# masafumiendo/benchnav

Hardware: AMD Instinct MI355X
Metric: MPPI solve-steps/sec (K=1024,T=50,256x256 map) (higher is better)
Workload: dtype f32

## Files before the change

### benchnav_amd/csrc/mppi_capi.cpp

```cpp
#include "../../include/benchnav_mppi.h"
#include "mppi_kernels.h"
#include "bn_host.h"
#include "astar_dwa.h"
#include "clrrt_view.h"

#include <algorithm>
#include <atomic>
#include <cmath>
#include <chrono>
#include <cstdarg>
#include <cstdio>
#include <cstdlib>
#include <cstring>
#include <cerrno>
#include <sys/stat.h>
#include <fcntl.h>
#include <sys/file.h>
#include <unistd.h>
#include <dlfcn.h>
#include <hsa/hsa.h>
#include <hsa/hsa_ext_amd.h>
#include <rccl/rccl.h>
#include <map>
#include <mutex>
// ... 83 lines not shown
    hipStream_t stream = nullptr;
    bool own_stream = false;
    int n_maps = 1;
    uint64_t solves = 0;
    bool map_set = false, goal_set = false;
    uint64_t map_epoch = 0, map_epoch_at_solve = 0;
    bool pipelined = false;
    bool slow_path = false;
    bool tail_pending = false;
    float *d_map = nullptr, *d_state = nullptr, *d_goal = nullptr, *d_mean = nullptr, *d_eps = nullptr;
    float *d_X = nullptr, *d_U = nullptr, *d_w = nullptr, *d_cost_out = nullptr;
    float *d_cost[kSlots] = {}, *d_part[kSlots] = {}, *d_state_copy[kSlots] = {};
    float *d_ustar = nullptr, *d_xstar = nullptr, *d_stats = nullptr, *d_scratch = nullptr;
    float *d_mean_used = nullptr;
    int *d_idx = nullptr;
    const float *last_eps = nullptr;
    bn::EpsMode last_mode = bn::kEpsPhilox;
    float *d_slip_std = nullptr;
    float *d_ustar2[kSlots] = {}, *d_stats2[kSlots] = {};
    bool ticket_overlap = false;
    std::vector<float> dwa_stage;
    int *d_ticket = nullptr;
    float *d_gpart = nullptr;
    int n_cus = 256;
    size_t resident_wgs = 1024;
    int n_streams = 1;
    hipStream_t xstream[kMaxStreams - 1] = {};
    std::vector<hipStream_t> parked;
    hipEvent_t ev_fork = nullptr, ev_join[kMaxStreams - 1] = {};
    hipEvent_t ev_guard[kMaxStreams] = {};
    unsigned long long *d_flags = nullptr;
    bool role_overlap = false;
    unsigned long long *d_gran[kSlots] = {};
    float *d_Xalt[kMaxStreams - 1] = {}, *d_Ualt[kMaxStreams - 1] = {};
    unsigned long long pub[kSlots] = {};
    unsigned long long tails = 0;
    bool prev_published = false;
    bool overlap_used = false;
    bool overlap_off = false;
    int *h_err = nullptr, *d_err = nullptr;
    unsigned long long *h_mail = nullptr, *d_mail = nullptr;
    float *d_mean_snap = nullptr;
    float *d_state_snaps = nullptr;
    size_t snap_cap = 0;
    size_t snap_slot = 0;
    bool arm_state_snap = false;
    struct BatchRec { int32_t n; const float *states; const float *eps; bn_noise_kind noise; int32_t eps_ring; int64_t eps_stride; bool episode; const float *z; };
    std::vector<BatchRec> journal;
    bool journal_lost = false;
    bool arm_snap = false;
    bool replaying = false, last_batch_overlapped = false;
    uint64_t journal_solves0 = 0, recoveries = 0;
    struct OvTune { double best[2] = {0, 0}, last[2] = {0, 0}, ema[2] = {0, 0}; int chosen = 0, explore = 0, slow_run = 0; uint64_t windows[2] = {0, 0}, since_explore = 0, switches = 0; } tune;
    struct OvSample { bool valid = false; std::chrono::steady_clock::time_point t{}; uint32_t prog = 0, enq = 0; } ov_sample;
    int run_mode = 0;
    float *self_out_copy = nullptr;
    const float *inline_state = nullptr;
    bool self_tail_launched = false;
    bool self_used = false;
    bool self_off = false;
    bool hp_enabled = false;
    hipStream_t hp_stream[2] = {};
    hipEvent_t hp_ev[2] = {};
    bool hp_unordered = false;
    int hp_unordered_q = 0;
    unsigned long long *h_req = nullptr, *d_req = nullptr;
// ... 620 lines not shown
    if (rc == BN_OK) {
        if (hipHostMalloc((void **)&h->h_mail, B * 2 * sizeof(unsigned long long), hipHostMallocMapped) != hipSuccess ||
            hipHostGetDevicePointer((void **)&h->d_mail, h->h_mail, 0) != hipSuccess) rc = fail(BN_ERR_HIP, "hipHostMalloc (first-action mailbox) failed");
        else std::memset(h->h_mail, 0, B * 2 * sizeof(unsigned long long));
    }
    p.mail = h->d_mail;
    if (h->lat_kernel && p.nblk <= 16 && 2 * p.T <= bn::kRolloutThreads && !exp_env("BN_NO_GRANULES"))
        for (int q = 0; q < kSlots; ++q) alloc(&h->d_gran[q], (B * (size_t)p.nblk * (2 + 2 * T) + 4 * B) * sizeof(unsigned long long));
    h->role_overlap = h->pipelined && !h->lat_kernel && !(cfg->flags & BN_FLAG_NO_OVERLAP);
    if (const char *e = exp_env("BN_ROLE_OVERLAP")) h->role_overlap = h->role_overlap && e[0] != '0';
    const bool ticket_det = !h->slow_path && !p.slip_on && !h->pipelined && !(cfg->flags & BN_FLAG_NO_PIPELINE) && p.nblk <= 1024 &&
                            bn::finish_lds_bytes(p) + 256 <= bn::rollout_lds_bytes(p);
    h->ticket_overlap = (ticket_det || (!(cfg->flags & BN_FLAG_NO_PIPELINE) && bn::sampled_fused(p))) && !(cfg->flags & BN_FLAG_NO_OVERLAP) &&
                        !exp_env("BN_NO_TICKET_OVERLAP");
    const bool may_overlap = (h->lat_kernel || h->role_overlap || h->ticket_overlap) && !(cfg->flags & BN_FLAG_NO_OVERLAP);
    if (may_overlap) {
        h->n_streams = 2;
        if (const char *e = exp_env("BN_OVERLAP_STREAMS")) h->n_streams = std::min(std::max(std::atoi(e), 2), kMaxStreams);
        for (int q = 0; q + 1 < h->n_streams; ++q) {
            if (h->d_X) alloc(&h->d_Xalt[q], B * (T + 1) * 3 * (size_t)p.Kp * 4);
            if (h->d_U) alloc(&h->d_Ualt[q], B * T * 2 * (size_t)p.Kp * 4);
        }
        h->snap_cap = std::max<size_t>(64, std::min<size_t>(4096, ((size_t)16 << 20) / ((size_t)B * 12)));
        alloc(&h->d_state_snaps, h->snap_cap * B * 3 * 4);
    }
    if (rc == BN_OK && may_overlap) {
        bool ok = hipEventCreateWithFlags(&h->ev_fork, hipEventDisableTiming) == hipSuccess;
        for (int q = 0; ok && q < h->n_streams; ++q) ok = hipEventCreateWithFlags(&h->ev_guard[q], hipEventDisableTiming) == hipSuccess;
        for (int q = 0; ok && q + 1 < h->n_streams; ++q)
            ok = hipStreamCreateWithFlags(&h->xstream[q], hipStreamNonBlocking) == hipSuccess &&
                 hipEventCreateWithFlags(&h->ev_join[q], hipEventDisableTiming) == hipSuccess;
        if (!ok) rc = fail(BN_ERR_HIP, "stream / event creation for overlapped launches failed");
    }
    if (p.slip_on) {
        alloc(&h->d_slip_std, (size_t)h->n_maps * p.G * p.G * 4);
        p.slip_std = h->d_slip_std;
        for (int q = 0; q < kSlots; ++q) {
            alloc(&h->d_ustar2[q], (size_t)p.B * p.T * 2 * 4);
            alloc(&h->d_stats2[q], (size_t)p.B * 2 * 4);
        }
        alloc(&h->d_ticket, (size_t)p.B * 65 * 4);
        alloc(&h->d_gpart, (size_t)p.B * 64 * (2 + 2 * p.T) * 4);
        p.ticket = h->d_ticket; p.gpart = h->d_gpart;
        h->ticket_mode = !h->slow_path && !(cfg->flags & BN_FLAG_NO_PIPELINE) && bn::sampled_fused(p);
    } else if (ticket_det) {
        for (int q = 0; q < kSlots; ++q) {
            alloc(&h->d_ustar2[q], (size_t)p.B * p.T * 2 * 4);
            alloc(&h->d_stats2[q], (size_t)p.B * 2 * 4);
        }
        alloc(&h->d_ticket, (size_t)p.B * 65 * 4);
        alloc(&h->d_gpart, (size_t)p.B * 64 * (2 + 2 * p.T) * 4);
        p.gpart = h->d_gpart;
        h->ticket_mode = true;
    }
    if (rc == BN_OK && !p.pow2) {
        unsigned long long *bad = h->d_flags + ((kSlots + 1) * B + 1) * bn::kFlagStride;
        const float d_max = std::max(p.x_hi - p.x0, p.y_hi - p.y0);
        unsigned long long n_bad = 1;
        if (!(std::isfinite(d_max) && d_max >= 0.0f) || bn::launch_quotient_check(p.res, p.inv_res, d_max, bad, nullptr) != hipSuccess ||
            hipMemcpy(&n_bad, bad, sizeof n_bad, hipMemcpyDeviceToHost) != hipSuccess) {
            (void)hipGetLastError();
            rc = fail(BN_ERR_HIP, "checking the cell-index quotient for resolution %g failed", (double)p.res);
        } else if (n_bad != 0) {
            rc = fail(BN_ERR_INVALID, "resolution %.9g: the correctly rounded three-instruction quotient disagrees with the division for %llu "
                                      "positions in [0, %g] (no such resolution was known: please report it); use a neighbouring value",
                      (double)p.res, n_bad, (double)d_max);
// ... 98 lines not shown
static void shard_comm_release(bn_mppi *h);

void bn_mppi_destroy(bn_mppi_t *h)
{
    if (!h) return;
    DeviceGuard guard(h->cfg.device_id);
    hp_cancel(h);
    (void)hipStreamSynchronize(h->stream);
    {
        std::lock_guard<std::mutex> lock(g_overlap_mu);
        auto it = g_overlap_owner.find(h->cfg.device_id);
        if (it != g_overlap_owner.end() && it->second == h) g_overlap_owner.erase(it);
        g_overlap_owners.store((int)g_overlap_owner.size(), std::memory_order_relaxed);
        auto &v = g_handles[h->cfg.device_id];
        v.erase(std::remove(v.begin(), v.end(), h), v.end());
    }
    for (hipEvent_t e : h->ev) (void)hipEventDestroy(e);
    if (h->shard_comm || h->shard_prepared) shard_comm_release(h);
    void *bufs[] = {h->d_map, h->d_state, h->d_goal, h->d_mean, h->d_eps, h->d_X, h->d_U, h->d_cost_out,
                    h->d_w, h->d_ustar , h->d_stats, h->d_scratch, h->d_idx, h->d_lat_mean, h->d_lat_std,
                    h->d_ep_states, h->d_ep_reward, h->d_env_state, h->d_ep_done, h->d_ep_action, h->d_slip_std,
                    h->d_ustar2[0], h->d_ustar2[1], h->d_ustar2[2], h->d_ustar2[3], h->d_stats2[0], h->d_stats2[1], h->d_stats2[2], h->d_stats2[3],
                    h->d_ticket, h->d_gpart, h->d_mean_used, h->d_ad_i, h->d_ad_state, h->d_ad_log,
                    h->d_cl_rover, h->d_cl_flags, h->d_cl_goal, h->d_cl_log};
    static_assert(kSlots == 4, "the list above names the four slots");
    for (void *b : bufs)
        if (b) (void)hipFree(b);
    if (h->d_flags) (void)hipFree(h->d_flags);
    if (h->h_cl_pending) (void)hipHostFree(h->h_cl_pending);
    for (hipEvent_t e : h->cl_ev)
        if (e) (void)hipEventDestroy(e);
    for (int q = 0; q < kSlots; ++q) {
        if (h->d_gran[q]) (void)hipFree(h->d_gran[q]);
        if (h->d_cost[q]) (void)hipFree(h->d_cost[q]);
        if (h->d_part[q]) (void)hipFree(h->d_part[q]);
        if (h->d_state_copy[q]) (void)hipFree(h->d_state_copy[q]);
    }
    for (int q = 0; q < kMaxStreams - 1; ++q) {
        if (h->d_Xalt[q]) (void)hipFree(h->d_Xalt[q]);
        if (h->d_Ualt[q]) (void)hipFree(h->d_Ualt[q]);
        if (h->xstream[q]) { (void)hipStreamSynchronize(h->xstream[q]); (void)hipStreamDestroy(h->xstream[q]); }
        if (h->ev_join[q]) (void)hipEventDestroy(h->ev_join[q]);
    }
    for (hipStream_t ps : h->parked) (void)hipStreamDestroy(ps);
    if (h->ev_fork) (void)hipEventDestroy(h->ev_fork);
    for (hipEvent_t e : h->ev_guard) if (e) (void)hipEventDestroy(e);
    if (h->h_pinned) (void)hipHostFree(h->h_pinned);
    if (h->h_err) (void)hipHostFree(h->h_err);
    if (h->h_mail) (void)hipHostFree(h->h_mail);
    if (h->h_req) (void)hipHostFree(h->h_req);
    if (h->req_bar) bar_free(h->req_bar);
    if (h->d_req_dev) (void)hipFree(h->d_req_dev);
    for (hipEvent_t e : h->hp_ev) if (e) (void)hipEventDestroy(e);
    if (h->d_mean_snap) (void)hipFree(h->d_mean_snap);
    if (h->d_state_snaps) (void)hipFree(h->d_state_snaps);
    if (h->own_stream && h->stream) (void)hipStreamDestroy(h->stream);
    delete h;
}

int bn_mppi_set_map(bn_mppi_t *h, int32_t instance, const float *risk, bn_mem_kind where)
{
    if (int rc = check_instance(h, instance, true)) return rc;
    if (!risk) return fail(BN_ERR_INVALID, "risk is null");
    BN_BIND(h);
    if (int rc = settle_point(h)) return rc;
    const size_t bytes = (size_t)h->p.G * h->p.G * 4;
// ... 282 lines not shown
        h->solves += 1;
        h->x_idx = 0;
        h->tail_pending = !p.self_tail;
        if (p.self_tail) h->prev_published = false;
        if (lone_self) h->last_batch_overlapped = false;
        return BN_OK;
    }
    if (!(h->ticket_overlap && overlap && !shard_rollout)) h->prev_published = false;
    p.have_prev = 0;
    p.mean_from_part = 0;
    p.tail_solve = p.solve;
    if (p.slip_on && !h->slip_std_set) return fail(BN_ERR_STATE, "bn_mppi_set_slip_std must precede solve in sampled-slip mode");
    if (h->ticket_mode && !shard_rollout) {
        p.have_prev = h->tail_pending ? 1 : 0;
        p.tail_merged = 1;
        p.tail_solve = p.solve - 1;
        p.ustar_cur = h->d_ustar2[cur3]; p.stats_cur = h->d_stats2[cur3];
        p.ustar_prev = h->d_ustar2[prev3]; p.stats_prev = h->d_stats2[prev3];
        p.ticket = h->d_ticket;
        hipStream_t st = h->stream;
        p.flag_tail = h->d_flags + kSlots * B * bn::kFlagStride;
        if (p.have_prev) { p.wait_tail = h->tails; h->tails += 1; }
        if (h->ticket_overlap && overlap) {
            p.flag_part = h->d_flags;
            p.err = h->d_err; p.err_dev = reinterpret_cast<int *>(h->d_flags + ((kSlots + 1) * B + 2) * bn::kFlagStride);
            if (h->arm_snap) { p.mean_snap = h->d_mean_snap; h->arm_snap = false; }
            p.cur_slot = cur3; p.prev_slot = prev3;
            p.wait_part = h->pub[prev3];
            if (alt_buffers) {
                if (h->d_Xalt[alt_buffers - 1]) p.X = h->d_Xalt[alt_buffers - 1];
                if (h->d_Ualt[alt_buffers - 1] && p.U) p.U = h->d_Ualt[alt_buffers - 1];
            }
            p.overlap = (h->prev_published && p.have_prev) ? 1 : 0;
            if (on_stream) st = on_stream;
            if (p.overlap) h->overlap_used = true;
            h->pub[cur3] += 1;
            h->prev_published = true;
        }
        if (p.slip_on) BN_HIP(bn::launch_rollout_sampled(p, mode, st));
        else BN_HIP(bn::launch_rollout(p, mode, st));
        if (prof_grouped) h->prof_in_group = (h->prof_in_group + 1) % kProfGroup;
        h->solves += 1;
        h->tail_pending = true;
        return BN_OK;
    }
    if (shard_rollout && h->shard_inplace) p.part = h->d_gathered + (size_t)h->shard_rank * p.nblk * (2 + 2 * T);
    if (p.slip_on) {
        BN_HIP(bn::launch_rollout_sampled(p, mode, h->stream));
    } else {
        if (h->slow_path) p.wave_kernel = 1;
        else if (!p.store_u) p.U = nullptr;
        BN_HIP(bn::launch_rollout(p, mode, h->stream));
    }
    if (prof) BN_HIP(hipEventRecord(ev[1], h->stream));
    if (shard_rollout) {
        if (prof) BN_HIP(hipEventRecord(ev[2], h->stream));
        h->solves += 1;
        h->tail_pending = false;
        h->shard_pending = true;
        return BN_OK;
    }
    p.state = p.state_copy;
    BN_HIP(bn::launch_finish(p, h->stream));
    if (prof) BN_HIP(hipEventRecord(ev[2], h->stream));
    h->solves += 1;
    h->tail_pending = false;
// ... 1489 lines not shown
```

### benchnav_amd/csrc/mppi_device.h

```cpp
#pragma once
#include "mppi_kernels.h"
#include "bn_device_math.h"

#include <math.h>
#include <algorithm>

namespace bn {

namespace {


constexpr int TU = kChunk;

#ifdef BN_EXPERIMENTS
#include "experiments.h"
#else
#define BN_STAMP(slot) do { } while (0)
#define BN_STAMP_ANY(slot) do { } while (0)
#define BN_WSTAMP(i) do { } while (0)
#define BN_TRACE_BEGIN() do { } while (0)
#define BN_TRACE_END() do { } while (0)
#define BN_TIMING_DO(...)
#define BN_SSTAMP(i) do { } while (0)
#endif
// ... 353 lines not shown
    for (int j = lane; j < 2 * p.T; j += 64) p.mean_snap[(size_t)b * 2 * p.T + j] = ml[j];
}

template <int SLEEP = 1>
__device__ __forceinline__ void wait_counter(const unsigned long long *ctr, unsigned long long need, const SolveParams &p)
{
    for (int it = 0; it < (1 << 23) / SLEEP + 1024; ++it) {
        if (__hip_atomic_load(ctr, __ATOMIC_RELAXED, __HIP_MEMORY_SCOPE_AGENT) >= need) return;
        __builtin_amdgcn_s_sleep(SLEEP);
    }
    raise_wait_expired(p, ctr, need);
}

__device__ __forceinline__ void publish_counter(unsigned long long *ctr, int tid)
{
    asm volatile("s_waitcnt vmcnt(0)" ::: "memory");
    __syncthreads();
    if (tid == 0) __hip_atomic_fetch_add(ctr, 1ull, __ATOMIC_RELAXED, __HIP_MEMORY_SCOPE_AGENT);
}

__device__ __forceinline__ void store_granule(unsigned long long *ptr, float v, uint32_t tag)
{
    __hip_atomic_store(ptr, ((unsigned long long)tag << 32) | (unsigned long long)__float_as_uint(v), __ATOMIC_RELAXED, __HIP_MEMORY_SCOPE_AGENT);
}
__device__ __forceinline__ void store_granule_host(unsigned long long *ptr, float v, uint32_t tag)
{
    __hip_atomic_store(ptr, ((unsigned long long)tag << 32) | (unsigned long long)__float_as_uint(v), __ATOMIC_RELAXED, __HIP_MEMORY_SCOPE_SYSTEM);
}
__device__ __forceinline__ float load_granule(const unsigned long long *ptr, uint32_t tag, bool &ok)
{
    const unsigned long long g = __hip_atomic_load(ptr, __ATOMIC_RELAXED, __HIP_MEMORY_SCOPE_AGENT);
    ok = ok && (uint32_t)(g >> 32) == tag;
    return __uint_as_float((uint32_t)g);
}

template <int NT, bool AGENT>
__device__ __forceinline__ void column_sums(const float *Ul, const float *el, int T, int tid, float *part,
                                            unsigned long long *grow = nullptr, uint32_t tag = 0)
{
    for (int it = tid; it < 8 * T; it += NT) {
        const int j = it >> 2, r = it & 3;
        const float *col = Ul + j * kUPad + 16 * r, *e = el + 16 * r;
        float acc = 0.0f;
#pragma unroll
        for (int q = 0; q < 16; ++q) acc = __builtin_fmaf(e[q], col[q], acc);
        asm volatile("s_nop 1\n\t"
                     "v_add_f32_dpp %0, %0, %0 quad_perm:[1,0,3,2] row_mask:0xf bank_mask:0xf\n\ts_nop 1\n\t"
                     "v_add_f32_dpp %0, %0, %0 quad_perm:[2,3,0,1] row_mask:0xf bank_mask:0xf\n\ts_nop 1"
                     : "+v"(acc));
        if (r == 0) {
            if (grow) store_granule(grow + 2 + j, acc, tag);
            if (AGENT) store_agent(part + 2 + j, acc); else part[2 + j] = acc;
        }
    }
}

template <int NT>
__device__ __forceinline__ float block_reduce(float v, float *red, int tid, bool is_max)
{
    v = is_max ? wave_max(v) : wave_sum(v);
    if ((tid & 63) == 0) red[tid >> 6] = v;
    __syncthreads();
    float r = red[0];
    for (int i = 1; i < NT / 64; ++i) r = is_max ? fmaxf(r, red[i]) : r + red[i];
    __syncthreads();
    return r;
// ... 507 lines not shown
            const float ck = ld<AGENT>(cost + k);
            st<AGENT>(cout + k, ck);
            st<AGENT>(wout + k, expf((-ck) / p.lambda_ - m) / S);
        }
    }
    if constexpr (NT == 64) {
        const float *cost = cost_all + (size_t)b * K;
        float *wout = p.w + (size_t)b * K;
        float *cout = p.cost_out + (size_t)b * K;
        for (int k = tid; k < K; k += 64) {
            const float ck = cost[k];
            cout[k] = ck;
            wout[k] = expf((-ck) / p.lambda_ - m) / S;
        }
    }
    BN_SSTAMP(4);
    __syncthreads();
    BN_SSTAMP(5);
    {
        float *Xg = p.xstar + (size_t)b * (T + 1) * 3;
        float *Xc = p.out_copy ? p.out_copy + (size_t)p.B * 2 * T + (size_t)b * (T + 1) * 3 : nullptr;
        for (int i = tid; i < 3 * (T + 1); i += NT) {
            const float v = xl[i];
            st<AGENT>(Xg + i, v);
            if (Xc) st<AGENT>(Xc + i, v);
        }
    }
    if (p.flag_tail) publish_counter(flag_ctr(p.flag_tail, b), tid);
    BN_SSTAMP(6);
}

constexpr int kTicketStride = 1 + 64;

template <int NT>
__device__ __forceinline__ void ticket_merge(const SolveParams &p, int b, int blk, float *scratch)
{
    const int T = p.T, tid = threadIdx.x, PS = 2 + 2 * p.T;
    float *us = scratch, *sc = us + 2 * T, *red = sc + p.nblk;
    int *flag = reinterpret_cast<int *>(red + 32);
    int *ticket = p.ticket + (size_t)b * kTicketStride;
    const float *part = p.part + (size_t)b * p.nblk * PS;
    const float *rows = part;
    int nrows = p.nblk;
    if (p.nblk > 64) {
        const int g = blk / kGroupRows, ng = (p.nblk + kGroupRows - 1) / kGroupRows;
        const int in_group = min(kGroupRows, p.nblk - g * kGroupRows);
        asm volatile("s_waitcnt vmcnt(0)" ::: "memory");
        __syncthreads();
        if (tid == 0) *flag = (atomicAdd(ticket + 1 + g, 1) == in_group - 1) ? 1 : 0;
        __syncthreads();
        if (!*flag) return;
        if (tid == 0) __hip_atomic_store(ticket + 1 + g, 0, __ATOMIC_RELAXED, __HIP_MEMORY_SCOPE_AGENT);
        float *grow = p.gpart + ((size_t)b * 64 + g) * PS;
        merge_group<true, true>(part, g * kGroupRows, in_group, T, tid & 63, tid >> 6, NT / 64, grow);
        rows = p.gpart + (size_t)b * 64 * PS;
        nrows = ng;
    }
    asm volatile("s_waitcnt vmcnt(0)" ::: "memory");
    __syncthreads();
    if (tid == 0) *flag = (atomicAdd(ticket, 1) == nrows - 1) ? 1 : 0;
    __syncthreads();
    if (!*flag) return;
    BN_STAMP_ANY(6);
    if (tid == 0) __hip_atomic_store(ticket, 0, __ATOMIC_RELAXED, __HIP_MEMORY_SCOPE_AGENT);
    float m, S;
    merge_partials<NT, true, false>(rows, nrows, T, us, sc, red, tid, m, S, false, MergeLoads{});
    const bool pubm = p.flag_part != nullptr;
    const bool spoiled = pubm && batch_spoiled(p);
    for (int j = tid; j < 2 * T; j += NT) {
        const size_t at = (size_t)b * 2 * T + j;
        if (pubm) {
            store_agent(p.ustar_cur + at, us[j]);
            if (spoiled) continue;
            if (p.mean_used) store_agent(p.mean_used + at, load_agent(p.mean + at));
            store_agent(p.mean + at, us[j]);
        } else {
            p.ustar_cur[at] = us[j];
            if (p.mean_used) p.mean_used[at] = p.mean[at];
            p.mean[at] = us[j];
        }
    }
    if (tid == 0) {
        if (pubm) { store_agent(p.stats_cur + b * 2 + 0, m); store_agent(p.stats_cur + b * 2 + 1, S); }
        else { p.stats_cur[b * 2 + 0] = m; p.stats_cur[b * 2 + 1] = S; }
    }
    if (pubm) publish_counter(flag_ctr(p.flag_part, p.cur_slot * p.B + b), tid);
    BN_STAMP_ANY(7);
}

#define BN_BAR() asm volatile("s_waitcnt lgkmcnt(0)\n\ts_barrier" ::: "memory")

template <int EPS, bool STORE_U, bool FRESH = false>
__device__ __forceinline__ void produce_pair(const SolveParams &p, const float *__restrict__ eps, int b, int kk, int t,
                                             uint64_t solve, const float *ml, float *Ul, float *Ub, size_t Kp, int lane)
{
    float e[4];
    const int t1 = min(t + 1, p.T - 1);
    if (EPS == kEpsPhilox) {
        philox_eps_pair<FRESH>(p.seed, solve, (uint32_t)b, (uint32_t)(kk + p.k0), (uint32_t)(t >> 1), e);
    } else if (EPS == kEpsKT2) {
        const float *row = eps + ((size_t)b * p.K + kk) * p.T * 2;
        const float2 v0 = *reinterpret_cast<const float2 *>(row + 2 * t);
        const float2 v1 = *reinterpret_cast<const float2 *>(row + 2 * t1);
        e[0] = v0.x; e[1] = v0.y; e[2] = v1.x; e[3] = v1.y;
    } else {
        const float *r0 = eps + ((size_t)b * p.T + t) * 2 * p.K;
        const float *r1 = eps + ((size_t)b * p.T + t1) * 2 * p.K;
        e[0] = r0[kk]; e[1] = r0[p.K + kk]; e[2] = r1[kk]; e[3] = r1[p.K + kk];
    }
#pragma unroll
    for (int s = 0; s < 2; ++s) {
        const int tt = t + s;
        if (tt < p.T) {
            const float u0 = clampf(ml[2 * tt] + p.sigma0 * e[2 * s], p.umin0, p.umax0);
            const float u1 = clampf(ml[2 * tt + 1] + p.sigma1 * e[2 * s + 1], p.umin1, p.umax1);
            Ul[(2 * tt) * kUPad + lane] = u0;
            Ul[(2 * tt + 1) * kUPad + lane] = u1;
            if (STORE_U) { float *Ut = Ub + (size_t)(2 * tt) * Kp; Ut[0] = u0; Ut[Kp] = u1; }
        }
// ... 56 lines not shown
```

### benchnav_amd/csrc/rollout_role.inc

```
#include "mppi_device.h"

#ifndef BN_ROLE_REF
#define BN_ROLE_REF false
#endif
#ifndef BN_ROLE_FRESH
#define BN_ROLE_FRESH false
#endif

namespace bn {

namespace {

template <int EPS, int GEO, bool LDSWIN, bool STORE_U, bool TICKET, bool REF>
__global__ __launch_bounds__(kRolloutThreads) void rollout_kernel(const SolveParams p)
{
    extern __shared__ __attribute__((aligned(16))) float smem[];
    BN_TRACE_BEGIN();
    const WgId wg = decode_wg(p);
    if (wg.idle) return;
    if (wg.aux) {
        if (p.aux_prio) __builtin_amdgcn_s_setprio(3);
        if (p.overlap) finish_body<GEO, LDSWIN, kRolloutThreads, false, true, false, REF>(p, wg.b, p.part_prev, p.cost_prev, p.state_prev, smem);
        else finish_body<GEO, LDSWIN, kRolloutThreads, false, false, false, REF>(p, wg.b, p.part_prev, p.cost_prev, p.state_prev, smem);
        BN_TRACE_END();
// ... 19 lines not shown
    const float *__restrict__ map = p.map + (size_t)b * p.map_stride;
    const float *__restrict__ eps = p.eps;
    const float *st_src = p.closed_loop ? p.state_prev : p.state;
    float sx = st_src[b * 3 + 0], sy = st_src[b * 3 + 1], sth = st_src[b * 3 + 2];
    const float gx = p.goal[b * 2 + 0], gy = p.goal[b * 2 + 1];
    const uint64_t solve = p.solve;
    BN_STAMP(0);

    const float *part_prev = p.part_prev + (size_t)b * p.nblk * (2 + 2 * T);
    const bool ov = p.overlap && p.mean_from_part;
    MergeLoads pre{};
    const bool pre_ok = p.mean_from_part && p.nblk <= 64 && !ov;
    if (pre_ok) pre = merge_issue(part_prev, p.nblk, T, tid);

    Win w{0, 0, 0.f, 0.f, 0.f, 0.f};
    if (LDSWIN && !p.closed_loop) {
        w = window_origin<GEO>(p, sx, sy);
        stage_window(win, map, w, p.WN, p.G, tid, kRolloutThreads);
    }
    if (ov) {
        if (tid == 0) wait_counter<16>(flag_ctr(p.flag_part, p.prev_slot * p.B + b), p.wait_part, p);
        __syncthreads();
        if (p.closed_loop) {
            sx = load_agent(st_src + b * 3 + 0); sy = load_agent(st_src + b * 3 + 1); sth = load_agent(st_src + b * 3 + 2);
        }
        float m_unused, S_unused;
        merge_partials<kRolloutThreads, true>(part_prev, p.nblk, T, ml, ring, ring + p.nblk, tid, m_unused, S_unused, false, pre);
        for (int j = tid; j < 2 * T; j += kRolloutThreads) mv[j] = ml[j] * ((j & 1) ? p.iv1 : p.iv0);
    } else if (p.mean_from_part) {
        float m_unused, S_unused;
        merge_partials<kRolloutThreads>(part_prev, p.nblk, T, ml, ring, ring + p.nblk, tid, m_unused, S_unused, pre_ok, pre);
        for (int j = tid; j < 2 * T; j += kRolloutThreads) mv[j] = ml[j] * ((j & 1) ? p.iv1 : p.iv0);
    } else if (TICKET && p.overlap) {
        if (tid == 0) wait_counter<16>(flag_ctr(p.flag_part, p.prev_slot * p.B + b), p.wait_part, p);
        __syncthreads();
        for (int j = tid; j < 2 * T; j += kRolloutThreads) {
            const float m = load_agent(p.mean + (size_t)b * 2 * T + j);
            ml[j] = m;
            mv[j] = m * ((j & 1) ? p.iv1 : p.iv0);
        }
    } else {
        for (int j = tid; j < 2 * T; j += kRolloutThreads) {
            const float m = p.mean[(size_t)b * 2 * T + j];
            ml[j] = m;
            mv[j] = m * ((j & 1) ? p.iv1 : p.iv0);
        }
    }
    if (p.closed_loop) {
        const EnvStep e = env_advance<GEO>(p, b, sx, sy, sth, ml[0], ml[1], p.env_z, (uint64_t)p.ep_index);
        sx = e.x; sy = e.y; sth = e.th;
        if (LDSWIN) {
            w = window_origin<GEO>(p, sx, sy);
            stage_window(win, map, w, p.WN, p.G, tid, kRolloutThreads);
        }
    }
    const bool pub = !TICKET && p.flag_part != nullptr;
    const bool tpub = TICKET && p.flag_part != nullptr;
    if (wg.blk == 0 && tid == 0) {
        if (pub || (TICKET && p.flag_part != nullptr)) { store_agent(p.state_copy + b * 3 + 0, sx); store_agent(p.state_copy + b * 3 + 1, sy); store_agent(p.state_copy + b * 3 + 2, sth); }
        else { p.state_copy[b * 3 + 0] = sx; p.state_copy[b * 3 + 1] = sy; p.state_copy[b * 3 + 2] = sth; }
        if (p.state_snap) { p.state_snap[b * 3 + 0] = sx; p.state_snap[b * 3 + 1] = sy; p.state_snap[b * 3 + 2] = sth; }
    }
    BN_BAR();
    if (p.mean_snap && wg.blk == 0 && wid == 0) snapshot_mean(p, b, ml, lane);

    const size_t Kp = (size_t)p.Kp;
    const bool lean = p.lean != 0;
    float *Xb = p.X + (size_t)b * (T + 1) * 3 * Kp + k;
    float *Ub = STORE_U ? p.U + (size_t)b * T * 2 * Kp + k : nullptr;

    if (wid < 4) {
#pragma unroll
        for (int q = 0; q < TU / 4; ++q) {
// ... 235 lines not shown
```

### benchnav_amd/csrc/rollout_sampled.hip

```cpp
#include "mppi_device.h"

namespace bn {

namespace {

constexpr int kSampledWaves = 8;
constexpr int kSampledThreads = 64 * kSampledWaves;

__host__ __device__ inline size_t sampled_lds_floats(int T, int WN)
{
    const size_t TP = (size_t)((T + 2) & ~1);
    return 4 * 64 * (size_t)(T + 1) + 2 * (size_t)WN * WN + 2 * 64 * TP + 2 * (size_t)T * kUPad + 4 * (size_t)T + 128;
}

template <int EPS, int GEO, bool STORE_U>
__global__ __launch_bounds__(kSampledThreads) void rollout_sampled_kernel(const SolveParams p)
{
    extern __shared__ __attribute__((aligned(16))) float smem[];
    const int T = p.T, K = p.K, WN2 = p.WN * p.WN;
    const int TP = (T + 2) & ~1;
    float4 *XL = reinterpret_cast<float4 *>(smem);
    float2 *win2 = reinterpret_cast<float2 *>(smem + 4 * 64 * (T + 1));
    float *Zt = reinterpret_cast<float *>(win2 + WN2), *Zc = Zt + 64 * TP;
    float *Ul = Zc + 64 * TP, *ml = Ul + 2 * T * kUPad, *mv = ml + 2 * T, *el = mv + 2 * T, *ad = el + 64;
    const WgId wg = decode_wg(p);
    if (wg.idle) return;
    const int tid = threadIdx.x, lane = tid & 63, b = wg.b;
    if (wg.aux) {
        if (p.overlap) finish_body<GEO, true, kSampledThreads, false, true>(p, b, nullptr, p.cost_prev, p.state_prev, smem);
        else finish_body<GEO, true, kSampledThreads>(p, b, nullptr, p.cost_prev, p.state_prev, smem);
        return;
    }
    const int wid = __builtin_amdgcn_readfirstlane(tid >> 6);
    const int k = wg.blk * 64 + lane;
    const bool active = k < K;
    const int kk = active ? k : K - 1;
    const float *__restrict__ mu = p.map + (size_t)b * p.map_stride;
    const float *__restrict__ sg = p.slip_std + (size_t)b * p.map_stride;
    const float sx = p.state[b * 3 + 0], sy = p.state[b * 3 + 1], sth = p.state[b * 3 + 2];
    const float gx = p.goal[b * 2 + 0], gy = p.goal[b * 2 + 1];
    const Win w = window_origin<GEO>(p, sx, sy);
    const size_t Kp = (size_t)p.Kp;
    float *Xb = p.X + (size_t)b * (T + 1) * 3 * Kp + k;
    float *Ub = STORE_U ? p.U + (size_t)b * T * 2 * Kp + k : nullptr;

    BN_STAMP(0);
    for (int e = tid; e < WN2; e += kSampledThreads) {
        const int r = e / p.WN, c = e - r * p.WN;
        const size_t g = (size_t)min(w.wy0 + r, p.G - 1) * p.G + min(w.wx0 + c, p.G - 1);
        win2[e] = make_float2(mu[g], sg[g]);
    }
    const bool ovs = p.overlap != 0;
    const bool tpub = p.flag_part != nullptr;
    if (!ovs)
    for (int j = tid; j < 2 * T; j += kSampledThreads) {
        const float m = p.mean[(size_t)b * 2 * T + j];
        ml[j] = m;
        mv[j] = m * ((j & 1) ? p.iv1 : p.iv0);
    }
    if (wg.blk == 0 && tid < 3) { if (tpub) store_agent(p.state_copy + b * 3 + tid, p.state[b * 3 + tid]); else p.state_copy[b * 3 + tid] = p.state[b * 3 + tid]; }
    if (p.state_snap && wg.blk == 0 && tid < 3) p.state_snap[b * 3 + tid] = p.state[b * 3 + tid];
    __syncthreads();

    {
        const int nE = (T + 1) >> 1, nS = TP >> 1;
        for (int q = nE + wid; q < nE + nS; q += kSampledWaves) {
            {
                const int r0 = 2 * (q - nE), r1 = r0 + 1;
                float z[4];
                if (p.zt) {
                    z[0] = r0 < T ? p.zt[((size_t)b * T + r0) * K + kk] : 0.0f;
                    z[1] = r1 < T ? p.zt[((size_t)b * T + r1) * K + kk] : 0.0f;
                    z[2] = r0 <= T ? p.zc[((size_t)b * (T + 1) + r0) * K + kk] : 0.0f;
                    z[3] = r1 <= T ? p.zc[((size_t)b * (T + 1) + r1) * K + kk] : 0.0f;
                } else {
                    philox_slip_block(p.seed, p.solve, (uint32_t)b, (uint32_t)(kk + p.k0), (uint32_t)(q - nE), z);
                }
                Zt[r0 * 64 + lane] = z[0]; Zt[r1 * 64 + lane] = z[1];
                Zc[r0 * 64 + lane] = z[2]; Zc[r1 * 64 + lane] = z[3];
            }
        }
        if (ovs) {
            if (tid == 0) wait_counter<16>(flag_ctr(p.flag_part, p.prev_slot * p.B + b), p.wait_part, p);
            __syncthreads();
            for (int j = tid; j < 2 * T; j += kSampledThreads) {
                const float m = load_agent(p.mean + (size_t)b * 2 * T + j);
                ml[j] = m;
                mv[j] = m * ((j & 1) ? p.iv1 : p.iv0);
            }
            __syncthreads();
        }
        if (p.mean_snap && wg.blk == 0 && wid == 0) snapshot_mean(p, b, ml, lane);
        for (int q = wid; q < nE; q += kSampledWaves) produce_pair<EPS, STORE_U>(p, p.eps, b, kk, 2 * q, p.solve, ml, Ul, Ub, Kp, lane);
    }
    __syncthreads();
    BN_STAMP(1);

    if (wid == 0) {
        SlipChain c;
        c.x = sx; c.y = sy; c.th = sth;
        sincos_spec(c.th, c.sn, c.cs);
        c.e = slip_cell_safe<GEO, true>(p, w, sx, sy);
        float xn, yn, tn;
        slip_chain_step<GEO, true>(p, win2, w, c, Ul[lane], Ul[kUPad + lane], Zt[lane], xn, yn, tn);
        XL[lane] = make_float4(xn, yn, tn, __int_as_float(c.e));
        int t = 1;
        for (; t + 4 <= T; t += 4) {
            float uq[4][3];
#pragma unroll
            for (int i = 0; i < 4; ++i) {
                uq[i][0] = Ul[(2 * (t + i)) * kUPad + lane]; uq[i][1] = Ul[(2 * (t + i) + 1) * kUPad + lane];
                uq[i][2] = Zt[(t + i) * 64 + lane];
            }
#pragma unroll
            for (int i = 0; i < 4; ++i) {
                slip_chain_step<GEO, false>(p, win2, w, c, uq[i][0], uq[i][1], uq[i][2], xn, yn, tn);
                __builtin_amdgcn_sched_barrier(0);
                XL[(t + i) * 64 + lane] = make_float4(xn, yn, tn, __int_as_float(c.e));
            }
        }
        for (; t < T; ++t) {
            slip_chain_step<GEO, false>(p, win2, w, c, Ul[(2 * t) * kUPad + lane], Ul[(2 * t + 1) * kUPad + lane], Zt[t * 64 + lane],
                                        xn, yn, tn);
            XL[t * 64 + lane] = make_float4(xn, yn, tn, __int_as_float(c.e));
        }
        XL[T * 64 + lane] = make_float4(c.x, c.y, c.th, __int_as_float(c.e));
    } else if (wid == 1) {
        double Ad = 0.0;
        for (int t = 0; t < T; ++t)
            Ad += (double)(p.lambda_ * (mv[2 * t] * Ul[(2 * t) * kUPad + lane] + mv[2 * t + 1] * Ul[(2 * t + 1) * kUPad + lane]));
        ad[lane] = (float)Ad;
    }
    __syncthreads();
    BN_STAMP(2);

    for (int t = wid; t <= T; t += kSampledWaves) {
        const float4 o = XL[t * 64 + lane];
        float *Xt = Xb + (size_t)(3 * t) * Kp;
        Xt[0] = o.x; Xt[Kp] = o.y; Xt[2 * Kp] = o.z;
        const float2 ms = win2[__float_as_int(o.w)];
        const float tc = trav_from_slip(ms.x, ms.y, Zc[t * 64 + lane]);
        const float dx = o.x - gx, dy = o.y - gy;
        Zc[t * 64 + lane] = sqrt_cr_normal(dx * dx + dy * dy) + (tc <= p.thr ? 1.0e4f : 0.0f);
    }
    __syncthreads();
    BN_STAMP(3);

    if (wid == 0) {
        double Sd = 0.0;
#pragma unroll 16
        for (int t = 0; t < T; ++t) Sd += (double)Zc[t * 64 + lane];
        const float cost = ((float)Sd + Zc[T * 64 + lane]) + ad[lane];
        if (active) { if (tpub) store_agent(p.cost + (size_t)b * K + k, cost); else p.cost[(size_t)b * K + k] = cost; }
        const float zz = active ? (-cost) / p.lambda_ : -INFINITY;
        const float zmax = wave_max(zz);
        const float e = active ? expf(zz - zmax) : 0.0f;
        const float esum = wave_sum(e);
        el[lane] = e;
        if (lane == 0) {
            float *part = p.part + ((size_t)b * p.nblk + wg.blk) * (2 + 2 * T);
            store_agent(part, zmax); store_agent(part + 1, esum);
        }
    }
    __syncthreads();
    column_sums<kSampledThreads, true>(Ul, el, T, tid, p.part + ((size_t)b * p.nblk + wg.blk) * (2 + 2 * T));
    BN_STAMP(5);
    if (p.ustar_cur) ticket_merge<kSampledThreads>(p, b, wg.blk, smem);
}

template <int EPS, int GEO, bool STORE_U>
__global__ __launch_bounds__(64) void rollout_sampled_global_kernel(const SolveParams p)
{
    extern __shared__ __attribute__((aligned(16))) float smem[];
    const int T = p.T, K = p.K;
    float *ml = smem, *mv = ml + 2 * T, *Ul = mv + 2 * T, *el = Ul + 2 * T * kUPad;
    const WgId wg = decode_wg(p);
    if (wg.idle) return;
    const int lane = threadIdx.x, b = wg.b;
    const int k = wg.blk * 64 + lane;
    const bool active = k < K;
    const int kk = active ? k : K - 1;
    const float *__restrict__ mu = p.map + (size_t)b * p.map_stride;
    const float *__restrict__ sg = p.slip_std + (size_t)b * p.map_stride;
    const float sx = p.state[b * 3 + 0], sy = p.state[b * 3 + 1], sth = p.state[b * 3 + 2];
    const float gx = p.goal[b * 2 + 0], gy = p.goal[b * 2 + 1];
    const Win w{0, 0, 0.f, 0.f, 0.f, 0.f};
    for (int j = lane; j < 2 * T; j += 64) {
        const float m = p.mean[(size_t)b * 2 * T + j];
        ml[j] = m;
        mv[j] = m * ((j & 1) ? p.iv1 : p.iv0);
    }
    if (wg.blk == 0 && lane < 3) p.state_copy[b * 3 + lane] = p.state[b * 3 + lane];
    if (p.state_snap && wg.blk == 0 && lane < 3) p.state_snap[b * 3 + lane] = p.state[b * 3 + lane];
    __syncthreads();
    const size_t Kp = (size_t)p.Kp;
    float *Xb = p.X + (size_t)b * (T + 1) * 3 * Kp + k;
// ... 159 lines not shown
```

Baseline: 106,200.

## Stream per-element mean granules and pipeline slip chain with cost consumers via LDS progress

```diff
diff --git a/benchnav_amd/csrc/mppi_capi.cpp b/benchnav_amd/csrc/mppi_capi.cpp
--- a/benchnav_amd/csrc/mppi_capi.cpp
+++ b/benchnav_amd/csrc/mppi_capi.cpp
@@ -139,6 +139,7 @@
     unsigned long long *d_flags = nullptr;
     bool role_overlap = false;
     unsigned long long *d_gran[kSlots] = {};
+    unsigned long long *d_ugran[kSlots] = {};
     float *d_Xalt[kMaxStreams - 1] = {}, *d_Ualt[kMaxStreams - 1] = {};
     unsigned long long pub[kSlots] = {};
     unsigned long long tails = 0;
@@ -825,6 +826,8 @@
                  hipEventCreateWithFlags(&h->ev_join[q], hipEventDisableTiming) == hipSuccess;
         if (!ok) rc = fail(BN_ERR_HIP, "stream / event creation for overlapped launches failed");
     }
+    if (h->ticket_overlap)
+        for (int q = 0; q < kSlots; ++q) alloc(&h->d_ugran[q], (size_t)p.B * p.T * 2 * sizeof(unsigned long long));
     if (p.slip_on) {
         alloc(&h->d_slip_std, (size_t)h->n_maps * p.G * p.G * 4);
         p.slip_std = h->d_slip_std;
@@ -989,6 +992,7 @@
         if (e) (void)hipEventDestroy(e);
     for (int q = 0; q < kSlots; ++q) {
         if (h->d_gran[q]) (void)hipFree(h->d_gran[q]);
+        if (h->d_ugran[q]) (void)hipFree(h->d_ugran[q]);
         if (h->d_cost[q]) (void)hipFree(h->d_cost[q]);
         if (h->d_part[q]) (void)hipFree(h->d_part[q]);
         if (h->d_state_copy[q]) (void)hipFree(h->d_state_copy[q]);
@@ -1337,6 +1341,8 @@
                 if (h->d_Ualt[alt_buffers - 1] && p.U) p.U = h->d_Ualt[alt_buffers - 1];
             }
             p.overlap = (h->prev_published && p.have_prev) ? 1 : 0;
+            p.gran = h->d_ugran[cur3];
+            p.gran_prev = p.overlap ? h->d_ugran[prev3] : nullptr;
             if (on_stream) st = on_stream;
             if (p.overlap) h->overlap_used = true;
             h->pub[cur3] += 1;
diff --git a/benchnav_amd/csrc/mppi_device.h b/benchnav_amd/csrc/mppi_device.h
--- a/benchnav_amd/csrc/mppi_device.h
+++ b/benchnav_amd/csrc/mppi_device.h
@@ -409,6 +409,26 @@
     const unsigned long long g = __hip_atomic_load(ptr, __ATOMIC_RELAXED, __HIP_MEMORY_SCOPE_AGENT);
     ok = ok && (uint32_t)(g >> 32) == tag;
     return __uint_as_float((uint32_t)g);
+}
+
+__device__ __forceinline__ void poll_mean_granules(const SolveParams &p, int b, int wid, int lane, float *ml, float *mv)
+{
+    const int n = 2 * p.T;
+    if (wid * 128 >= n) return;
+    const unsigned long long *ug = p.gran_prev + (size_t)b * n;
+    const uint32_t tag = (uint32_t)p.solve;
+    const int j0 = wid * 128 + lane, j1 = j0 + 64;
+    const unsigned long long *a0 = ug + min(j0, n - 1), *a1 = ug + min(j1, n - 1);
+    unsigned long long g0 = 0, g1 = 0;
+    bool got = false;
+    for (int it = 0; it < (1 << 22); ++it) {
+        g0 = __hip_atomic_load(a0, __ATOMIC_RELAXED, __HIP_MEMORY_SCOPE_AGENT);
+        g1 = __hip_atomic_load(a1, __ATOMIC_RELAXED, __HIP_MEMORY_SCOPE_AGENT);
+        if (__all((uint32_t)(g0 >> 32) == tag && (uint32_t)(g1 >> 32) == tag)) { got = true; break; }
+    }
+    if (!got && lane == 0) raise_wait_expired(p, nullptr, 266);
+    if (j0 < n) { const float m = __uint_as_float((uint32_t)g0); ml[j0] = m; mv[j0] = m * ((j0 & 1) ? p.iv1 : p.iv0); }
+    if (j1 < n) { const float m = __uint_as_float((uint32_t)g1); ml[j1] = m; mv[j1] = m * ((j1 & 1) ? p.iv1 : p.iv0); }
 }
 
 template <int NT, bool AGENT>
@@ -982,59 +1002,92 @@
 
 constexpr int kTicketStride = 1 + 64;
 
+struct TicketLate {
+    int overlap, prev_slot, cur_slot, B;
+    unsigned long long wait_part;
+    unsigned long long *flag_part, *gran;
+    const unsigned long long *gran_prev;
+    int *ticket, *err_dev;
+    float *gpart, *ustar_cur, *stats_cur, *mean, *mean_used;
+};
+__device__ __forceinline__ TicketLate ticket_late_params()
+{
+    typedef const __attribute__((address_space(4))) SolveParams *kargs_t;
+    kargs_t kp = (kargs_t)__builtin_amdgcn_kernarg_segment_ptr();
+    asm volatile("" : "+s"(kp));
+    TicketLate l;
+    l.overlap = kp->overlap; l.prev_slot = kp->prev_slot; l.B = kp->B; l.wait_part = kp->wait_part;
+    l.flag_part = kp->flag_part; l.gran = kp->gran; l.gran_prev = kp->gran_prev; l.cur_slot = kp->cur_slot;
+    l.ticket = kp->ticket; l.err_dev = kp->err_dev; l.gpart = kp->gpart; l.ustar_cur = kp->ustar_cur; l.stats_cur = kp->stats_cur;
+    l.mean = kp->mean; l.mean_used = kp->mean_used;
+    return l;
+}
+
 template <int NT>
 __device__ __forceinline__ void ticket_merge(const SolveParams &p, int b, int blk, float *scratch)
 {
     const int T = p.T, tid = threadIdx.x, PS = 2 + 2 * p.T;
     float *us = scratch, *sc = us + 2 * T, *red = sc + p.nblk;
     int *flag = reinterpret_cast<int *>(red + 32);
-    int *ticket = p.ticket + (size_t)b * kTicketStride;
+    const TicketLate lp = ticket_late_params();
+    int *ticket = lp.ticket + (size_t)b * kTicketStride;
     const float *part = p.part + (size_t)b * p.nblk * PS;
     const float *rows = part;
     int nrows = p.nblk;
+    const bool late_count = lp.overlap && lp.gran_prev != nullptr;
     if (p.nblk > 64) {
         const int g = blk / kGroupRows, ng = (p.nblk + kGroupRows - 1) / kGroupRows;
         const int in_group = min(kGroupRows, p.nblk - g * kGroupRows);
         asm volatile("s_waitcnt vmcnt(0)" ::: "memory");
         __syncthreads();
-        if (tid == 0) *flag = (atomicAdd(ticket + 1 + g, 1) == in_group - 1) ? 1 : 0;
+        if (tid == 0) {
+            if (late_count) wait_counter<16>(flag_ctr(lp.flag_part, lp.prev_slot * lp.B + b), lp.wait_part, p);
+            *flag = (atomicAdd(ticket + 1 + g, 1) == in_group - 1) ? 1 : 0;
+        }
         __syncthreads();
         if (!*flag) return;
         if (tid == 0) __hip_atomic_store(ticket + 1 + g, 0, __ATOMIC_RELAXED, __HIP_MEMORY_SCOPE_AGENT);
-        float *grow = p.gpart + ((size_t)b * 64 + g) * PS;
+        float *grow = lp.gpart + ((size_t)b * 64 + g) * PS;
         merge_group<true, true>(part, g * kGroupRows, in_group, T, tid & 63, tid >> 6, NT / 64, grow);
-        rows = p.gpart + (size_t)b * 64 * PS;
+        rows = lp.gpart + (size_t)b * 64 * PS;
         nrows = ng;
     }
     asm volatile("s_waitcnt vmcnt(0)" ::: "memory");
     __syncthreads();
-    if (tid == 0) *flag = (atomicAdd(ticket, 1) == nrows - 1) ? 1 : 0;
+    if (tid == 0) {
+        if (late_count && p.nblk <= 64) wait_counter<16>(flag_ctr(lp.flag_part, lp.prev_slot * lp.B + b), lp.wait_part, p);
+        *flag = (atomicAdd(ticket, 1) == nrows - 1) ? 1 : 0;
+    }
     __syncthreads();
     if (!*flag) return;
     BN_STAMP_ANY(6);
     if (tid == 0) __hip_atomic_store(ticket, 0, __ATOMIC_RELAXED, __HIP_MEMORY_SCOPE_AGENT);
+    const bool pubm = lp.flag_part != nullptr;
+    float old_mean = 0.0f;
+    if (pubm && lp.mean_used && tid < 2 * T) old_mean = load_agent(lp.mean + (size_t)b * 2 * T + tid);
     float m, S;
     merge_partials<NT, true, false>(rows, nrows, T, us, sc, red, tid, m, S, false, MergeLoads{});
-    const bool pubm = p.flag_part != nullptr;
-    const bool spoiled = pubm && batch_spoiled(p);
+    const bool spoiled = pubm && lp.err_dev != nullptr && __hip_atomic_load(lp.err_dev, __ATOMIC_RELAXED, __HIP_MEMORY_SCOPE_AGENT) != 0;
+    const uint32_t utag = (uint32_t)p.solve + 1u;
     for (int j = tid; j < 2 * T; j += NT) {
         const size_t at = (size_t)b * 2 * T + j;
         if (pubm) {
-            store_agent(p.ustar_cur + at, us[j]);
+            if (lp.gran) store_granule(lp.gran + at, us[j], utag);
+            store_agent(lp.ustar_cur + at, us[j]);
             if (spoiled) continue;
-            if (p.mean_used) store_agent(p.mean_used + at, load_agent(p.mean + at));
-            store_agent(p.mean + at, us[j]);
+            if (lp.mean_used) store_agent(lp.mean_used + at, j == tid ? old_mean : load_agent(lp.mean + at));
+            store_agent(lp.mean + at, us[j]);
         } else {
-            p.ustar_cur[at] = us[j];
-            if (p.mean_used) p.mean_used[at] = p.mean[at];
-            p.mean[at] = us[j];
+            lp.ustar_cur[at] = us[j];
+            if (lp.mean_used) lp.mean_used[at] = lp.mean[at];
+            lp.mean[at] = us[j];
         }
     }
     if (tid == 0) {
-        if (pubm) { store_agent(p.stats_cur + b * 2 + 0, m); store_agent(p.stats_cur + b * 2 + 1, S); }
-        else { p.stats_cur[b * 2 + 0] = m; p.stats_cur[b * 2 + 1] = S; }
-    }
-    if (pubm) publish_counter(flag_ctr(p.flag_part, p.cur_slot * p.B + b), tid);
+        if (pubm) { store_agent(lp.stats_cur + b * 2 + 0, m); store_agent(lp.stats_cur + b * 2 + 1, S); }
+        else { lp.stats_cur[b * 2 + 0] = m; lp.stats_cur[b * 2 + 1] = S; }
+    }
+    if (pubm) publish_counter(flag_ctr(lp.flag_part, lp.cur_slot * lp.B + b), tid);
     BN_STAMP_ANY(7);
 }
 
diff --git a/benchnav_amd/csrc/rollout_role.inc b/benchnav_amd/csrc/rollout_role.inc
--- a/benchnav_amd/csrc/rollout_role.inc
+++ b/benchnav_amd/csrc/rollout_role.inc
@@ -75,13 +75,7 @@
         merge_partials<kRolloutThreads>(part_prev, p.nblk, T, ml, ring, ring + p.nblk, tid, m_unused, S_unused, pre_ok, pre);
         for (int j = tid; j < 2 * T; j += kRolloutThreads) mv[j] = ml[j] * ((j & 1) ? p.iv1 : p.iv0);
     } else if (TICKET && p.overlap) {
-        if (tid == 0) wait_counter<16>(flag_ctr(p.flag_part, p.prev_slot * p.B + b), p.wait_part, p);
-        __syncthreads();
-        for (int j = tid; j < 2 * T; j += kRolloutThreads) {
-            const float m = load_agent(p.mean + (size_t)b * 2 * T + j);
-            ml[j] = m;
-            mv[j] = m * ((j & 1) ? p.iv1 : p.iv0);
-        }
+        poll_mean_granules(p, b, wid, lane, ml, mv);
     } else {
         for (int j = tid; j < 2 * T; j += kRolloutThreads) {
             const float m = p.mean[(size_t)b * 2 * T + j];
diff --git a/benchnav_amd/csrc/rollout_sampled.hip b/benchnav_amd/csrc/rollout_sampled.hip
--- a/benchnav_amd/csrc/rollout_sampled.hip
+++ b/benchnav_amd/csrc/rollout_sampled.hip
@@ -6,6 +6,8 @@
 
 constexpr int kSampledWaves = 8;
 constexpr int kSampledThreads = 64 * kSampledWaves;
+constexpr int kSampledConsumers = kSampledWaves - 2;
+typedef __attribute__((address_space(3))) volatile int sl_vint;
 
 __host__ __device__ inline size_t sampled_lds_floats(int T, int WN)
 {
@@ -22,7 +24,8 @@
     float4 *XL = reinterpret_cast<float4 *>(smem);
     float2 *win2 = reinterpret_cast<float2 *>(smem + 4 * 64 * (T + 1));
     float *Zt = reinterpret_cast<float *>(win2 + WN2), *Zc = Zt + 64 * TP;
-    float *Ul = Zc + 64 * TP, *ml = Ul + 2 * T * kUPad, *mv = ml + 2 * T, *el = mv + 2 * T, *ad = el + 64;
+    float *Ul = Zc + 64 * TP, *ml = Ul + 2 * T * kUPad, *mv = ml + 2 * T, *el = mv + 2 * T;
+    int *prog = reinterpret_cast<int *>(el + 64);
     const WgId wg = decode_wg(p);
     if (wg.idle) return;
     const int tid = threadIdx.x, lane = tid & 63, b = wg.b;
@@ -60,6 +63,7 @@
     }
     if (wg.blk == 0 && tid < 3) { if (tpub) store_agent(p.state_copy + b * 3 + tid, p.state[b * 3 + tid]); else p.state_copy[b * 3 + tid] = p.state[b * 3 + tid]; }
     if (p.state_snap && wg.blk == 0 && tid < 3) p.state_snap[b * 3 + tid] = p.state[b * 3 + tid];
+    if (tid < 1 + kSampledConsumers) prog[tid] = 0;
     __syncthreads();
 
     {
@@ -81,21 +85,38 @@
             }
         }
         if (ovs) {
-            if (tid == 0) wait_counter<16>(flag_ctr(p.flag_part, p.prev_slot * p.B + b), p.wait_part, p);
+            for (int q = wid; q < nE; q += kSampledWaves) {
+                float e[4];
+                noise_pair<EPS>(p, b, kk, 2 * q, e);
+#pragma unroll
+                for (int s = 0; s < 2; ++s)
+                    if (2 * q + s < T) { Ul[(4 * q + 2 * s) * kUPad + lane] = e[2 * s]; Ul[(4 * q + 2 * s + 1) * kUPad + lane] = e[2 * s + 1]; }
+            }
+            poll_mean_granules(p, b, wid, lane, ml, mv);
             __syncthreads();
-            for (int j = tid; j < 2 * T; j += kSampledThreads) {
-                const float m = load_agent(p.mean + (size_t)b * 2 * T + j);
-                ml[j] = m;
-                mv[j] = m * ((j & 1) ? p.iv1 : p.iv0);
-            }
-            __syncthreads();
-        }
-        if (p.mean_snap && wg.blk == 0 && wid == 0) snapshot_mean(p, b, ml, lane);
-        for (int q = wid; q < nE; q += kSampledWaves) produce_pair<EPS, STORE_U>(p, p.eps, b, kk, 2 * q, p.solve, ml, Ul, Ub, Kp, lane);
+            if (p.mean_snap && wg.blk == 0 && wid == 0) snapshot_mean(p, b, ml, lane);
+            for (int q = wid; q < nE; q += kSampledWaves) {
+#pragma unroll
+                for (int s = 0; s < 2; ++s) {
+                    const int tt = 2 * q + s;
+                    if (tt < T) {
+                        const float u0 = clampf(ml[2 * tt] + p.sigma0 * Ul[(2 * tt) * kUPad + lane], p.umin0, p.umax0);
+                        const float u1 = clampf(ml[2 * tt + 1] + p.sigma1 * Ul[(2 * tt + 1) * kUPad + lane], p.umin1, p.umax1);
+                        Ul[(2 * tt) * kUPad + lane] = u0;
+                        Ul[(2 * tt + 1) * kUPad + lane] = u1;
+                        if (STORE_U) { float *Ut = Ub + (size_t)(2 * tt) * Kp; Ut[0] = u0; Ut[Kp] = u1; }
+                    }
+                }
+            }
+        } else {
+            if (p.mean_snap && wg.blk == 0 && wid == 0) snapshot_mean(p, b, ml, lane);
+            for (int q = wid; q < nE; q += kSampledWaves) produce_pair<EPS, STORE_U>(p, p.eps, b, kk, 2 * q, p.solve, ml, Ul, Ub, Kp, lane);
+        }
     }
     __syncthreads();
     BN_STAMP(1);
 
+    sl_vint *cprog = (sl_vint *)prog;
     if (wid == 0) {
         SlipChain c;
         c.x = sx; c.y = sy; c.th = sth;
@@ -104,6 +125,7 @@
         float xn, yn, tn;
         slip_chain_step<GEO, true>(p, win2, w, c, Ul[lane], Ul[kUPad + lane], Zt[lane], xn, yn, tn);
         XL[lane] = make_float4(xn, yn, tn, __int_as_float(c.e));
+        asm volatile("" ::: "memory"); *cprog = 1;
         int t = 1;
         for (; t + 4 <= T; t += 4) {
             float uq[4][3];
@@ -118,39 +140,33 @@
                 __builtin_amdgcn_sched_barrier(0);
                 XL[(t + i) * 64 + lane] = make_float4(xn, yn, tn, __int_as_float(c.e));
             }
+            asm volatile("" ::: "memory"); *cprog = t + 4;
         }
         for (; t < T; ++t) {
             slip_chain_step<GEO, false>(p, win2, w, c, Ul[(2 * t) * kUPad + lane], Ul[(2 * t + 1) * kUPad + lane], Zt[t * 64 + lane],
                                         xn, yn, tn);
             XL[t * 64 + lane] = make_float4(xn, yn, tn, __int_as_float(c.e));
+            asm volatile("" ::: "memory"); *cprog = t + 1;
         }
         XL[T * 64 + lane] = make_float4(c.x, c.y, c.th, __int_as_float(c.e));
+        asm volatile("" ::: "memory"); *cprog = T + 1;
+        BN_STAMP(2);
     } else if (wid == 1) {
         double Ad = 0.0;
         for (int t = 0; t < T; ++t)
             Ad += (double)(p.lambda_ * (mv[2 * t] * Ul[(2 * t) * kUPad + lane] + mv[2 * t + 1] * Ul[(2 * t + 1) * kUPad + lane]));
-        ad[lane] = (float)Ad;
-    }
-    __syncthreads();
-    BN_STAMP(2);
-
-    for (int t = wid; t <= T; t += kSampledWaves) {
-        const float4 o = XL[t * 64 + lane];
-        float *Xt = Xb + (size_t)(3 * t) * Kp;
-        Xt[0] = o.x; Xt[Kp] = o.y; Xt[2 * Kp] = o.z;
-        const float2 ms = win2[__float_as_int(o.w)];
-        const float tc = trav_from_slip(ms.x, ms.y, Zc[t * 64 + lane]);
-        const float dx = o.x - gx, dy = o.y - gy;
-        Zc[t * 64 + lane] = sqrt_cr_normal(dx * dx + dy * dy) + (tc <= p.thr ? 1.0e4f : 0.0f);
-    }
-    __syncthreads();
-    BN_STAMP(3);
-
-    if (wid == 0) {
         double Sd = 0.0;
-#pragma unroll 16
-        for (int t = 0; t < T; ++t) Sd += (double)Zc[t * 64 + lane];
-        const float cost = ((float)Sd + Zc[T * 64 + lane]) + ad[lane];
+        for (int t = 0;;) {
+            int avail = T + 1;
+#pragma unroll
+            for (int j = 0; j < kSampledConsumers; ++j) avail = min(avail, j + kSampledConsumers * ((sl_vint *)prog)[1 + j]);
+            asm volatile("" ::: "memory");
+            const int upto = min(avail, T);
+            for (; t < upto; ++t) Sd += (double)Zc[t * 64 + lane];
+            if (avail > T) break;
+            __builtin_amdgcn_s_sleep(1);
+        }
+        const float cost = ((float)Sd + Zc[T * 64 + lane]) + (float)Ad;
         if (active) { if (tpub) store_agent(p.cost + (size_t)b * K + k, cost); else p.cost[(size_t)b * K + k] = cost; }
         const float zz = active ? (-cost) / p.lambda_ : -INFINITY;
         const float zmax = wave_max(zz);
@@ -161,7 +177,24 @@
             float *part = p.part + ((size_t)b * p.nblk + wg.blk) * (2 + 2 * T);
             store_agent(part, zmax); store_agent(part + 1, esum);
         }
-    }
+    } else {
+        const int cw = wid - 2;
+        int done = 0;
+        for (int t = cw; t <= T; t += kSampledConsumers) {
+            while (*cprog <= t) __builtin_amdgcn_s_sleep(1);
+            asm volatile("" ::: "memory");
+            const float4 o = XL[t * 64 + lane];
+            float *Xt = Xb + (size_t)(3 * t) * Kp;
+            Xt[0] = o.x; Xt[Kp] = o.y; Xt[2 * Kp] = o.z;
+            const float2 ms = win2[__float_as_int(o.w)];
+            const float tc = trav_from_slip(ms.x, ms.y, Zc[t * 64 + lane]);
+            const float dx = o.x - gx, dy = o.y - gy;
+            Zc[t * 64 + lane] = sqrt_cr_normal(dx * dx + dy * dy) + (tc <= p.thr ? 1.0e4f : 0.0f);
+            asm volatile("" ::: "memory");
+            ((sl_vint *)prog)[1 + cw] = ++done;
+        }
+    }
+    BN_STAMP(3);
     __syncthreads();
     column_sums<kSampledThreads, true>(Ul, el, T, tid, p.part + ((size_t)b * p.nblk + wg.blk) * (2 + 2 * T));
     BN_STAMP(5);
```

New measurement: 104,700. 1.4% lower.
